# facebookresearch/rela

Hardware: AMD Instinct MI355X
Metric: env-steps/s (Ape-X Atari 84x84x4, actor tick + learner grad-step) (higher is better)
Workload: dtype f32 (f32 operands as 3 exact bf16 parts on bf16 MFMA; f32-accurate); 1 GPU; Ape-X DQN 80x80 envs/GPU, actor+learner on one MI355X, replay 2^20, B=512, A=18, n=3; device-resident static frames; parallelism=single

## Files before the change

### rela_amd/csrc/ffnet.hip

```cpp
#include <atomic>
#include <cstdlib>

#include "common.h"
#include "gemm_bf16s.h"
#include "gemm_f32emu.h"
#include "gemm_s3.h"
#include "conv_img_s3.h"
#include "conv12_s3.h"
#include "ffnet_layout.h"
#include "ffnet_plan.h"
#include "gemm_lds.h"
#include "param_layout.h"
#include "prof.h"

namespace rela_amd {

typedef float f32x4 __attribute__((ext_vector_type(4)));

struct FFNetDev {
  uint4* B1 = nullptr;
  float* b1 = nullptr;
  float *B2 = nullptr, *b2 = nullptr;
  float *B3 = nullptr, *b3 = nullptr;
  float *Bf = nullptr, *bf = nullptr;
// ... 1451 lines not shown
  const int64_t p = (int64_t)blockIdx.x * (blockDim.x >> 6) + (threadIdx.x >> 6);
  if (p >= pixels) return;
  const int c = threadIdx.x & 63;
  uint8_t* r = rec + p * 256;
  const uint16_t hi = reinterpret_cast<const uint16_t*>(r)[c], lo = reinterpret_cast<const uint16_t*>(r)[64 + c];
  const float v = bf16_to_f32(hi) + bf16_to_f32(lo);
  __builtin_amdgcn_wave_barrier();
  asm volatile("s_waitcnt vmcnt(0)" ::: "memory");
  reinterpret_cast<float*>(r)[c] = v;
}

using TileFcSmall = gemm::TileCfg<128, 64, 4, 2, false>;
struct ProbFcFwd : gemm::ProbBase {
  const float *a3, *wt;
  float* part;
  __device__ float4 loadA(int m, int k) const {
    return m < M ? *reinterpret_cast<const float4*>(a3 + (size_t)m * 3136 + k) : make_float4(0.f, 0.f, 0.f, 0.f);
  }
  __device__ float4 loadB(int k, int n) const { return *reinterpret_cast<const float4*>(wt + (size_t)k * 512 + n); }
  __device__ void store(int z, int m, int n, float v) const { part[((size_t)z * M + m) * 512 + n] = v; }
};

__global__ void fc_reduce(const float* __restrict__ part, int splits, int N, const float* __restrict__ bias,
                          float* __restrict__ h) {
  const int idx = blockIdx.x * blockDim.x + threadIdx.x;
  if (idx >= N * 128) return;
  const int n4 = (idx & 127) * 4;
  const size_t off = (size_t)(idx >> 7) * 512 + n4;
  float4 s = *reinterpret_cast<const float4*>(bias + n4);
  for (int z = 0; z < splits; ++z) {
    const float4 v = *reinterpret_cast<const float4*>(part + (size_t)z * N * 512 + off);
    s.x += v.x, s.y += v.y, s.z += v.z, s.w += v.w;
  }
  *reinterpret_cast<float4*>(h + off) =
// ... 1071 lines not shown
```

### rela_amd/csrc/gemm_bf16x3.h

```cpp
#pragma once
#include <hip/hip_runtime.h>

#include <type_traits>

#include "common.h"
#include "gemm_lds.h"
#include "prof.h"

namespace rela_amd {
namespace gemm3 {

typedef float f32x4 __attribute__((ext_vector_type(4)));
typedef float f32x2 __attribute__((ext_vector_type(2)));
typedef __bf16 bf16x8 __attribute__((ext_vector_type(8)));
typedef __bf16 bf16x2 __attribute__((ext_vector_type(2)));
typedef short s16x4 __attribute__((ext_vector_type(4)));
typedef s16x4 __attribute__((address_space(3))) * lds_s16x4_ptr;

constexpr int kT = 512;
constexpr int BK = 32;

__device__ __forceinline__ int krow(int k) {
  const int g = k >> 3, j = k & 7;
  return j < 4 ? 4 * g + j : 16 + 4 * g + (j - 4);
// ... 65 lines not shown
    return bz < gm.gz;
  }
  bx = (i / gm.gy) * 8 + xcd, by = i % gm.gy, bz = 0;
  return bx < gm.gx;
}

template <class T, class P>
__global__ __launch_bounds__(kT) void gemm_bf16x3(const P p, const GridMap gm) {
  extern __shared__ __attribute__((aligned(16))) uint8_t smem[];
  int bx, by, bz;
  if (!grid_map(gm, bx, by, bz)) return;
  const int tid = threadIdx.x;
  const int wave = tid >> 6, lane = tid & 63;
  const int li = lane & 15, g = lane >> 4;
  const int wm = wave / T::WN, wn = wave % T::WN;
  const int m0 = by * T::BM, n0 = bx * T::BN;
  const int nch = (p.K + BK - 1) / BK;
  const int c0 = bz * p.kslice;
  const int c1 = min(nch, c0 + p.kslice);

  constexpr int D = 4;
  float4 ra[D][T::A_IT], rb[D][T::B_IT];
  auto gload = [&](int ch, auto set) {
    constexpr int S = decltype(set)::value;
    const int k0 = ch * BK;
#pragma unroll
    for (int j = 0; j < T::A_IT; ++j) {
      const int idx = min(tid + j * kT, T::A_V4 - 1);
      if constexpr (T::AMC) {
        const int kr = idx / (T::BM / 4), q = idx % (T::BM / 4);
        ra[S][j] = p.loadA(k0 + kr, m0 + 4 * q);
      } else {
        const int r = idx >> 3, q = idx & 7;
        ra[S][j] = p.loadA(m0 + r, k0 + 4 * q);
      }
    }
#pragma unroll
    for (int j = 0; j < T::B_IT; ++j) {
      const int idx = min(tid + j * kT, T::B_V4 - 1);
      const int kr = idx / (T::BN / 4), q = idx % (T::BN / 4);
      rb[S][j] = p.loadB(k0 + kr, n0 + 4 * q);
    }
  };
  auto sstore = [&](int buf, auto set) {
    constexpr int S = decltype(set)::value;
    uint8_t* base = smem + buf * T::BUF;
#pragma unroll
    for (int j = 0; j < T::A_IT; ++j) {
      const int idx = min(tid + j * kT, T::A_V4 - 1);
      uint2 hi, mid, lo;
      if constexpr (T::PARTS == 3) split4x3(ra[S][j], hi, mid, lo);
      else split4(ra[S][j], hi, lo);
      int off;
      if constexpr (T::AMC) {
        const int kr = idx / (T::BM / 4), q = idx % (T::BM / 4);
        off = krow(kr) * T::LDA + q * 8;
      } else {
        const int r = idx >> 3, q = idx & 7;
        off = r * T::LDA + q * 8;
      }
      *reinterpret_cast<uint2*>(base + off) = hi;
      if constexpr (T::PARTS == 3) *reinterpret_cast<uint2*>(base + T::A_HALF + off) = mid;
      *reinterpret_cast<uint2*>(base + (T::PARTS - 1) * T::A_HALF + off) = lo;
    }
    uint8_t* bb = base + T::PARTS * T::A_HALF;
#pragma unroll
    for (int j = 0; j < T::B_IT; ++j) {
      const int idx = min(tid + j * kT, T::B_V4 - 1);
      const int kr = idx / (T::BN / 4), q = idx % (T::BN / 4);
      uint2 hi, mid, lo;
      if constexpr (T::PARTS == 3) split4x3(rb[S][j], hi, mid, lo);
      else split4(rb[S][j], hi, lo);
      const int off = krow(kr) * T::LDB + q * 8;
      *reinterpret_cast<uint2*>(bb + off) = hi;
      if constexpr (T::BPARTS == 3) *reinterpret_cast<uint2*>(bb + T::B_HALF + off) = mid;
      if constexpr (T::BPARTS > 1) *reinterpret_cast<uint2*>(bb + (T::BPARTS - 1) * T::B_HALF + off) = lo;
    }
  };

  const int tr_off = (4 * g + (li >> 2));
  auto frag_tr = [&](const uint8_t* img, int ld, int col0) -> bf16x8 {
    const uint8_t* a0 = img + tr_off * ld + (col0 + 4 * (li & 3)) * 2;
    const s16x4 x = __builtin_amdgcn_ds_read_tr16_b64_v4i16((lds_s16x4_ptr)(a0));
    const s16x4 y = __builtin_amdgcn_ds_read_tr16_b64_v4i16((lds_s16x4_ptr)(a0 + 16 * ld));
    typedef short s16x8 __attribute__((ext_vector_type(8)));
    const s16x8 z = {x[0], x[1], x[2], x[3], y[0], y[1], y[2], y[3]};
    return __builtin_bit_cast(bf16x8, z);
  };
  auto frag_row = [&](const uint8_t* img, int row) -> bf16x8 {
    return __builtin_bit_cast(bf16x8, *reinterpret_cast<const uint4*>(img + row * T::LDA + g * 16));
  };

  f32x4 acc[T::TM][T::TN];
  f32x4 accs[T::PARTS == 3 ? T::TM : 1][T::PARTS == 3 ? T::TN : 1];
#pragma unroll
  for (int t = 0; t < T::TM; ++t)
#pragma unroll
    for (int u = 0; u < T::TN; ++u) {
      acc[t][u] = f32x4{0.f, 0.f, 0.f, 0.f};
      if constexpr (T::PARTS == 3) accs[t][u] = f32x4{0.f, 0.f, 0.f, 0.f};
    }

  using S0 = std::integral_constant<int, 0>;
  using S1 = std::integral_constant<int, 1>;
  using S2 = std::integral_constant<int, 2>;
  using S3 = std::integral_constant<int, 3>;
  if (c0 < c1) gload(c0, S0{});
  if (c0 + 1 < c1) gload(c0 + 1, S1{});
  if (c0 + 2 < c1) gload(c0 + 2, S2{});
  if (c0 + 3 < c1) gload(c0 + 3, S3{});
  if (c0 < c1) sstore(0, S0{});
  __syncthreads();
  auto step = [&](int cur, auto cs, auto ns) {
    const int buf = (cur - c0) & 1;
    if (cur + D < c1) gload(cur + D, cs);
    const uint8_t* base = smem + buf * T::BUF;
    const uint8_t* bb = base + T::PARTS * T::A_HALF;
    bf16x8 bp[T::TN][T::BPARTS];
#pragma unroll
    for (int u = 0; u < T::TN; ++u) {
      const int col0 = (wn * T::TN + u) * 16;
#pragma unroll
      for (int q = 0; q < T::BPARTS; ++q) bp[u][q] = frag_tr(bb + q * T::B_HALF, T::LDB, col0);
    }
#pragma unroll
    for (int t = 0; t < T::TM; ++t) {
      const int row0 = (wm * T::TM + t) * 16;
      bf16x8 ap[T::PARTS];
#pragma unroll
      for (int q = 0; q < T::PARTS; ++q) {
// ... 8 lines not shown
          acc[t][u] = __builtin_amdgcn_mfma_f32_16x16x32_bf16(ap[0], bp[u][0], acc[t][u], 0, 0, 0);
        } else if constexpr (T::BPARTS == 1) {
          accs[t][u] = __builtin_amdgcn_mfma_f32_16x16x32_bf16(ap[2], bp[u][0], accs[t][u], 0, 0, 0);
          accs[t][u] = __builtin_amdgcn_mfma_f32_16x16x32_bf16(ap[1], bp[u][0], accs[t][u], 0, 0, 0);
          acc[t][u] = __builtin_amdgcn_mfma_f32_16x16x32_bf16(ap[0], bp[u][0], acc[t][u], 0, 0, 0);
        } else {
          accs[t][u] = __builtin_amdgcn_mfma_f32_16x16x32_bf16(ap[2], bp[u][0], accs[t][u], 0, 0, 0);
          accs[t][u] = __builtin_amdgcn_mfma_f32_16x16x32_bf16(ap[0], bp[u][2], accs[t][u], 0, 0, 0);
          accs[t][u] = __builtin_amdgcn_mfma_f32_16x16x32_bf16(ap[1], bp[u][1], accs[t][u], 0, 0, 0);
          accs[t][u] = __builtin_amdgcn_mfma_f32_16x16x32_bf16(ap[1], bp[u][0], accs[t][u], 0, 0, 0);
          accs[t][u] = __builtin_amdgcn_mfma_f32_16x16x32_bf16(ap[0], bp[u][1], accs[t][u], 0, 0, 0);
          acc[t][u] = __builtin_amdgcn_mfma_f32_16x16x32_bf16(ap[0], bp[u][0], acc[t][u], 0, 0, 0);
        }
      }
    }
    if (cur + 1 < c1) sstore(buf ^ 1, ns);
    __syncthreads();
  };
  for (int base = c0; base < c1; base += D) {
    step(base, S0{}, S1{});
    if (base + 1 < c1) step(base + 1, S1{}, S2{});
    if (base + 2 < c1) step(base + 2, S2{}, S3{});
    if (base + 3 < c1) step(base + 3, S3{}, S0{});
  }

#pragma unroll
  for (int t = 0; t < T::TM; ++t)
#pragma unroll
    for (int u = 0; u < T::TN; ++u)
#pragma unroll
      for (int r = 0; r < 4; ++r) {
        const int m = m0 + (wm * T::TM + t) * 16 + g * 4 + r;
        const int n = n0 + (wn * T::TN + u) * 16 + li;
        if (m < p.M && n < p.N) {
          if constexpr (T::PARTS == 3) p.store(bz, m, n, acc[t][u][r] + accs[t][u][r]);
          else p.store(bz, m, n, acc[t][u][r]);
        }
      }
}

template <class T, class P>
int launch_gemm(P p, int splits, hipStream_t s, const char* name) {
  static const hipError_t attr_set = hipFuncSetAttribute(reinterpret_cast<const void*>(&gemm_bf16x3<T, P>),
                                                         hipFuncAttributeMaxDynamicSharedMemorySize, T::LDS_BYTES);
  RELA_HIP(attr_set);
  const int nch = ceil_div(p.K, BK);
  p.kslice = ceil_div(nch, splits);
  ProfScope prof(name, s);
// ... 18 lines not shown
```

### rela_amd/csrc/gemm_lds.h

```cpp
#pragma once
#include <hip/hip_runtime.h>

#include <type_traits>

#include "common.h"
#include "prof.h"

namespace rela_amd {
namespace gemm {

typedef float f32x4 __attribute__((ext_vector_type(4)));
constexpr int kLT = 512;
constexpr int BK = 32;

__device__ __forceinline__ float4 zero4() { return make_float4(0.f, 0.f, 0.f, 0.f); }
__device__ __forceinline__ float4 ld4(const float* p) { return *reinterpret_cast<const float4*>(p); }

template <int BM_, int BN_, int WM_, int WN_, bool AMC_>
struct TileCfg {
  static constexpr int BM = BM_, BN = BN_, WM = WM_, WN = WN_;
  static constexpr bool AMC = AMC_;
  static_assert(WM * WN == 8, "8 wavefronts per block");
  static constexpr int TM = BM / 16 / WM, TN = BN / 16 / WN;
  static_assert(TM >= 1 && TN >= 1, "tile too small for the wave grid");
  static constexpr int LDA = AMC ? BM + 16 : BK + 2;
  static constexpr int A_FLOATS = AMC ? BK * LDA : BM * LDA;
  static constexpr int LDB = BN + 16;
  static constexpr int B_FLOATS = BK * LDB;
  static constexpr int A_V4 = BM * BK / 4, B_V4 = BN * BK / 4;
  static constexpr int A_IT = (A_V4 + kLT - 1) / kLT, B_IT = (B_V4 + kLT - 1) / kLT;
};

template <class P, class = void>
struct fold_chunks {
  static constexpr int value = 0;
};
template <class P>
struct fold_chunks<P, std::void_t<decltype(P::kFoldChunks)>> {
  static constexpr int value = P::kFoldChunks;
};

template <class T, class P>
__global__ __launch_bounds__(kLT) void gemm_lds(const P p) {
  __shared__ __attribute__((aligned(16))) float sA[2][T::A_FLOATS];
  __shared__ __attribute__((aligned(16))) float sB[2][T::B_FLOATS];
  const int tid = threadIdx.x;
  const int wave = tid >> 6, lane = tid & 63;
  const int li = lane & 15, kk = lane >> 4;
  const int wm = wave / T::WN, wn = wave % T::WN;
  const int m0 = blockIdx.y * T::BM, n0 = blockIdx.x * T::BN;
  const int nch = (p.K + BK - 1) / BK;
  const int c0 = blockIdx.z * p.kslice;
  const int c1 = min(nch, c0 + p.kslice);

  float4 ra[T::A_IT], rb[T::B_IT];
  auto gload = [&](int ch) {
    const int k0 = ch * BK;
#pragma unroll
    for (int j = 0; j < T::A_IT; ++j) {
      const int idx = tid + j * kLT;
      if (idx < T::A_V4) {
        if constexpr (T::AMC) {
          const int kr = idx / (T::BM / 4), q = idx % (T::BM / 4);
          ra[j] = p.loadA(k0 + kr, m0 + 4 * q);
        } else {
          const int r = idx >> 3, q = idx & 7;
          ra[j] = p.loadA(m0 + r, k0 + 4 * q);
        }
      }
    }
#pragma unroll
    for (int j = 0; j < T::B_IT; ++j) {
      const int idx = tid + j * kLT;
      if (idx < T::B_V4) {
        const int kr = idx / (T::BN / 4), q = idx % (T::BN / 4);
        rb[j] = p.loadB(k0 + kr, n0 + 4 * q);
      }
    }
  };
  auto sstore = [&](int buf) {
#pragma unroll
    for (int j = 0; j < T::A_IT; ++j) {
      const int idx = tid + j * kLT;
      if (idx < T::A_V4) {
        if constexpr (T::AMC) {
          const int kr = idx / (T::BM / 4), q = idx % (T::BM / 4);
          *reinterpret_cast<float4*>(&sA[buf][kr * T::LDA + 4 * q]) = ra[j];
        } else {
          const int r = idx >> 3, q = idx & 7;
          float* d = &sA[buf][r * T::LDA + 4 * q];
          *reinterpret_cast<float2*>(d) = make_float2(ra[j].x, ra[j].y);
          *reinterpret_cast<float2*>(d + 2) = make_float2(ra[j].z, ra[j].w);
        }
      }
    }
#pragma unroll
    for (int j = 0; j < T::B_IT; ++j) {
      const int idx = tid + j * kLT;
      if (idx < T::B_V4) {
        const int kr = idx / (T::BN / 4), q = idx % (T::BN / 4);
        *reinterpret_cast<float4*>(&sB[buf][kr * T::LDB + 4 * q]) = rb[j];
      }
    }
  };

  f32x4 acc[T::TM][T::TN];
#pragma unroll
  for (int t = 0; t < T::TM; ++t)
#pragma unroll
    for (int u = 0; u < T::TN; ++u) acc[t][u] = f32x4{0.f, 0.f, 0.f, 0.f};
  constexpr int FOLD = fold_chunks<P>::value;
  f32x4 tot[FOLD ? T::TM : 1][FOLD ? T::TN : 1];
  if constexpr (FOLD > 0) {
#pragma unroll
    for (int t = 0; t < T::TM; ++t)
#pragma unroll
      for (int u = 0; u < T::TN; ++u) tot[t][u] = f32x4{0.f, 0.f, 0.f, 0.f};
  }

  if (c0 < c1) {
    gload(c0);
    sstore(0);
  }
  __syncthreads();
  for (int ch = c0; ch < c1; ++ch) {
    const int buf = (ch - c0) & 1;
    if (ch + 1 < c1) gload(ch + 1);
#pragma unroll
    for (int ks = 0; ks < BK / 4; ++ks) {
      float a[T::TM], b[T::TN];
#pragma unroll
      for (int t = 0; t < T::TM; ++t) {
        const int row = (wm * T::TM + t) * 16 + li;
        a[t] = T::AMC ? sA[buf][(4 * ks + kk) * T::LDA + row] : sA[buf][row * T::LDA + 4 * ks + kk];
      }
#pragma unroll
      for (int u = 0; u < T::TN; ++u) b[u] = sB[buf][(4 * ks + kk) * T::LDB + (wn * T::TN + u) * 16 + li];
#pragma unroll
      for (int t = 0; t < T::TM; ++t)
#pragma unroll
        for (int u = 0; u < T::TN; ++u) acc[t][u] = __builtin_amdgcn_mfma_f32_16x16x4f32(a[t], b[u], acc[t][u], 0, 0, 0);
    }
    if constexpr (FOLD > 0) {
      if ((ch - c0 + 1) % FOLD == 0) {
#pragma unroll
        for (int t = 0; t < T::TM; ++t)
#pragma unroll
          for (int u = 0; u < T::TN; ++u) {
            tot[t][u] += acc[t][u];
            acc[t][u] = f32x4{0.f, 0.f, 0.f, 0.f};
          }
      }
    }
    if (ch + 1 < c1) sstore(buf ^ 1);
    __syncthreads();
  }

#pragma unroll
  for (int t = 0; t < T::TM; ++t)
#pragma unroll
    for (int u = 0; u < T::TN; ++u)
#pragma unroll
      for (int r = 0; r < 4; ++r) {
        const int m = m0 + (wm * T::TM + t) * 16 + kk * 4 + r;
        const int n = n0 + (wn * T::TN + u) * 16 + li;
        if (m < p.M && n < p.N) {
          if constexpr (FOLD > 0) p.store(blockIdx.z, m, n, tot[t][u][r]);
          else p.store(blockIdx.z, m, n, acc[t][u][r]);
        }
      }
}

struct ProbBase {
  int M, N, K, kslice;
};

template <class T, class P>
void launch_gemm(P p, int splits, hipStream_t s, const char* name) {
  const int nch = ceil_div(p.K, BK);
  p.kslice = ceil_div(nch, splits);
  ProfScope prof(name, s);
  note_launch("gemm_lds (f32)");
  hipLaunchKernelGGL((gemm_lds<T, P>), dim3(ceil_div(p.N, T::BN), ceil_div(p.M, T::BM), splits), dim3(kLT), 0, s, p);
}

}
}
```

### rela_amd/csrc/learner_common.h

```cpp
#pragma once
#include <cmath>
#include <cstring>
#include <vector>

#include "common.h"
#include "ffnet_layout.h"
#include "gemm_lds.h"
#include "gemm_bf16x3.h"
#include "param_layout.h"
#include "prof.h"
#include "value_rescale.h"
#include "dgrad_conv_bf16.h"
#include "wgrad_conv1_bf16.h"
#include "wgrad_conv2_bf16.h"
#include "wgrad_conv3_bf16.h"

namespace rela_amd {
namespace {

using namespace gemm;

using TileDgrad = TileCfg<128, 64, 4, 2, false>;
using TileWfc = TileCfg<128, 64, 4, 2, true>;
using TileW64 = TileCfg<64, 64, 2, 4, true>;
// ... 4 lines not shown
using Tile3Wfc = gemm3::TileCfg<128, 64, 4, 2, true>;
using Tile3W64 = gemm3::TileCfg<64, 64, 2, 4, true>;
using Tile3W32 = gemm3::TileCfg<32, 64, 2, 4, true>;
inline bool gemm_bf16x3_on() { return true; }
using Tile6Dgrad = gemm3::TileCfg<128, 64, 4, 2, false, 3>;
using Tile6Wfc = gemm3::TileCfg<128, 64, 4, 2, true, 3>;
using Tile6W64 = gemm3::TileCfg<64, 64, 2, 4, true, 3>;
using Tile6W32 = gemm3::TileCfg<32, 64, 2, 4, true, 3>;
using Tile6W32U8 = gemm3::SinglePartB<Tile6W32>;


struct ProbHeadDgrad : ProbBase {
  const float *d_ha, *a_w, *v_w, *h;
  float* d_h;
  int A;
  __device__ float4 loadA(int m, int k) const { return m < M ? ld4(d_ha + (size_t)m * 32 + k) : zero4(); }
  __device__ float4 loadB(int k, int n) const {
    if (k < A) return ld4(a_w + (size_t)k * 512 + n);
    if (k == 31) return ld4(v_w + n);
    return zero4();
  }
  __device__ void store(int, int m, int n, float v) const {
    const size_t i = (size_t)m * 512 + n;
    d_h[i] = h[i] > 0.f ? v : 0.f;
  }
};

struct ProbHeadWgradPart : ProbBase {
  const float *d_ha, *h;
  float* part;
  __device__ float4 loadA(int b, int m) const { return b < K ? ld4(d_ha + (size_t)b * 32 + m) : zero4(); }
  __device__ float4 loadB(int b, int n) const { return b < K ? ld4(h + (size_t)b * 512 + n) : zero4(); }
  __device__ void store(int z, int m, int n, float v) const { part[((size_t)z * 32 + m) * 512 + n] = v; }
};
__global__ void head_wgrad_reduce(const float* __restrict__ part, int splits, int A, float* __restrict__ g_a_w,
                                  float* __restrict__ g_v_w) {
  const int idx = blockIdx.x * blockDim.x + threadIdx.x;
  if (idx >= 32 * 512) return;
  const int m = idx >> 9, n = idx & 511;
  if (m >= A && m != 31) return;
  float s = 0.f;
#pragma unroll 8
  for (int z = 0; z < splits; ++z) s += part[(size_t)z * (32 * 512) + idx];
  if (m < A) g_a_w[(size_t)m * 512 + n] = s;
  else g_v_w[n] = s;
}

struct ProbHeadWgrad : ProbBase {
  const float *d_ha, *h;
  float *g_a_w, *g_v_w;
  int A;
  __device__ float4 loadA(int b, int m) const { return b < K ? ld4(d_ha + (size_t)b * 32 + m) : zero4(); }
  __device__ float4 loadB(int b, int n) const { return b < K ? ld4(h + (size_t)b * 512 + n) : zero4(); }
  __device__ void store(int, int m, int n, float v) const {
    if (m < A) g_a_w[(size_t)m * 512 + n] = v;
    else if (m == 31) g_v_w[n] = v;
  }
};

struct ProbFcDgrad : ProbBase {
  const float *d_h, *wfcp, *a3;
  float* d_a3;
  __device__ float4 loadA(int m, int k) const { return m < M ? ld4(d_h + (size_t)m * 512 + k) : zero4(); }
  __device__ float4 loadB(int k, int n) const { return ld4(wfcp + (size_t)k * 3136 + n); }
  __device__ void store(int, int m, int n, float v) const {
    const size_t i = (size_t)m * 3136 + n;
    d_a3[i] = a3[i] > 0.f ? v : 0.f;
  }
};

struct ProbFcWgrad : ProbBase {
  const float *d_h, *a3;
  float* g_fc_w;
  __device__ float4 loadA(int b, int m) const { return b < K ? ld4(d_h + (size_t)b * 512 + m) : zero4(); }
  __device__ float4 loadB(int b, int n) const { return b < K ? ld4(a3 + (size_t)b * 3136 + n) : zero4(); }
  __device__ void store(int, int m, int n, float v) const {
    const int pos = n >> 6, c = n & 63;
    g_fc_w[(size_t)m * 3136 + c * 49 + pos] = v;
  }
};

struct ProbDgrad3 : ProbBase {
  static constexpr int kFoldChunks = 2;
  const float *d_out, *wp, *a2;
  float* d_a2;
  __device__ float4 loadA(int m, int k) const {
    if (m >= M) return zero4();
    const int b = m / 81, pix = m - b * 81;
    const int y = pix / 9, x = pix - y * 9;
    const int tap = k >> 6, oc = k & 63;
    const int kh = tap / 3, kw = tap - kh * 3;
    const int oy = y - kh, ox = x - kw;
    if ((unsigned)oy >= 7u || (unsigned)ox >= 7u) return zero4();
    return ld4(d_out + ((size_t)b * 49 + oy * 7 + ox) * 64 + oc);
  }
  __device__ float4 loadB(int k, int n) const { return ld4(wp + (size_t)(k & 63) * 576 + (k >> 6) * 64 + n); }
  __device__ void store(int, int m, int n, float v) const {
    const size_t i = (size_t)m * 64 + n;
    d_a2[i] = a2[i] > 0.f ? v : 0.f;
  }
};

struct ProbDgrad2 : ProbBase {
  static constexpr int kFoldChunks = 2;
  const float *d_out, *wp, *a1;
  float* d_a1;
  __device__ float4 loadA(int m, int k) const {
    if (m >= M) return zero4();
    const int b = m / 100, pix = m - b * 100;
    const int yh = pix / 10, xh = pix - yh * 10;
    const int t = k >> 6, oc = k & 63;
    const int oy = yh - (t >> 1), ox = xh - (t & 1);
    if ((unsigned)oy >= 9u || (unsigned)ox >= 9u) return zero4();
    return ld4(d_out + ((size_t)b * 81 + oy * 9 + ox) * 64 + oc);
  }
  __device__ float4 loadB(int k, int n) const {
    const int cls = n >> 5, t = k >> 6;
    const int kh = (t & 2) + (cls >> 1), kw = 2 * (t & 1) + (cls & 1);
    return ld4(wp + (size_t)(k & 63) * 512 + (kh * 4 + kw) * 32 + (n & 31));
  }
  __device__ void store(int, int m, int n, float v) const {
    const int cls = n >> 5;
    const int b = m / 100, pix = m - b * 100;
    const int yh = pix / 10, xh = pix - yh * 10;
    const size_t i = ((size_t)b * 400 + (2 * yh + (cls >> 1)) * 20 + 2 * xh + (cls & 1)) * 32 + (n & 31);
    d_a1[i] = a1[i] > 0.f ? v : 0.f;
  }
};

template <int OC, int CIN, int KH, int KW, int STRIDE, int OH, int OW, int IH, int IW>
struct ProbConvWgrad : ProbBase {
  const float *d_out, *in;
  float* part;
  __device__ float4 loadA(int k, int m) const { return k < K ? ld4(d_out + (size_t)k * OC + m) : zero4(); }
  __device__ float4 loadB(int k, int n) const {
    if (k >= K) return zero4();
    const int b = k / (OH * OW), pos = k - b * (OH * OW);
    const int oy = pos / OW, ox = pos - oy * OW;
    const int r = n / CIN, c = n - r * CIN;
    const int kh = r / KW, kw = r - kh * KW;
    return ld4(in + (((size_t)b * IH + oy * STRIDE + kh) * IW + ox * STRIDE + kw) * CIN + c);
  }
  __device__ void store(int z, int m, int n, float v) const { part[((size_t)z * M + m) * N + n] = v; }
};
using ProbW3 = ProbConvWgrad<64, 64, 3, 3, 1, 7, 7, 9, 9>;
using ProbW2 = ProbConvWgrad<64, 32, 4, 4, 2, 9, 9, 20, 20>;

struct ProbW1 : ProbBase {
  const float* d_out;
  const uint8_t* obs;
  float* part;
  __device__ float4 loadA(int k, int m) const { return k < K ? ld4(d_out + (size_t)k * 32 + m) : zero4(); }
  __device__ float4 loadB(int k, int n) const {
    if (k >= K) return zero4();
    const int b = k / 400, pos = k - b * 400;
    const int oy = pos / 20, ox = pos - oy * 20;
    const int c = n >> 6, kh = (n >> 3) & 7, kw = n & 7;
    const uint32_t d = *reinterpret_cast<const uint32_t*>(obs + (size_t)b * 28224 + c * 7056 + (oy * 4 + kh) * 84 +
                                                          ox * 4 + kw);
    return make_float4((float)(d & 0xff), (float)((d >> 8) & 0xff), (float)((d >> 16) & 0xff), (float)(d >> 24));
  }
  __device__ void store(int z, int m, int n, float v) const { part[((size_t)z * M + m) * N + n] = v; }
};


enum { kRedConv1 = 0, kRedConv2 = 1, kRedConv3 = 2 };
__global__ void reduce_splits(const float* __restrict__ part, int splits, int M, int N, int mode,
                              float* __restrict__ out) {
  const int idx = blockIdx.x * blockDim.x + threadIdx.x;
  if (idx >= M * N) return;
  const int m = idx / N, n = idx - m * N;
  float s = 0.f;
#pragma unroll 8
  for (int z = 0; z < splits; ++z) s += part[((size_t)z * M + m) * N + n];
  if (mode == kRedConv1) {
// ... 564 lines not shown
```

### rela_amd/csrc/learner_r2d2.hip

```cpp
#include "gemm_bf16s.h"
#include "learner_common.h"

using namespace rela_amd;

namespace rela_amd {
namespace {

constexpr int kHid = 512, kGates = 2048, kFeat = 3136;
constexpr int kRecSplitF = 4;
constexpr int kRecSplitB = 8;

using TileRows = TileCfg<128, 64, 4, 2, false>;
using TileRec = TileCfg<64, 64, 2, 4, false>;
using TileWg = TileCfg<128, 64, 4, 2, true>;
using TileW32r = TileCfg<32, 64, 2, 4, true>;

struct ProbGateX : ProbBase {
  const float *a3, *wihT, *bias;
  float* gx;
  __device__ float4 loadA(int m, int k) const { return m < M ? ld4(a3 + (size_t)m * kFeat + k) : zero4(); }
  __device__ float4 loadB(int k, int n) const { return ld4(wihT + (size_t)k * kGates + n); }
  __device__ void store(int, int m, int n, float v) const { gx[(size_t)m * kGates + n] = v + bias[n]; }
};
struct ProbRecFwd : ProbBase {
  const float *h, *whhT;
  float* part;
  __device__ float4 loadA(int m, int k) const { return m < M ? ld4(h + (size_t)m * kHid + k) : zero4(); }
  __device__ float4 loadB(int k, int n) const { return ld4(whhT + (size_t)k * kGates + n); }
  __device__ void store(int z, int m, int n, float v) const { part[((size_t)z * M + m) * kGates + n] = v; }
};
struct ProbRecBwd : ProbBase {
  const float *dg, *whh;
  float* part;
  __device__ float4 loadA(int m, int k) const { return m < M ? ld4(dg + (size_t)m * kGates + k) : zero4(); }
  __device__ float4 loadB(int k, int n) const { return ld4(whh + (size_t)k * kHid + n); }
  __device__ void store(int z, int m, int n, float v) const { part[((size_t)z * M + m) * kHid + n] = v; }
};
struct ProbWhh : ProbBase {
  const float *dg, *hprev;
  float* out;
  __device__ float4 loadA(int r, int m) const { return r < K ? ld4(dg + (size_t)r * kGates + m) : zero4(); }
  __device__ float4 loadB(int r, int n) const { return r < K ? ld4(hprev + (size_t)r * kHid + n) : zero4(); }
  __device__ void store(int, int m, int n, float v) const { out[(size_t)m * kHid + n] = v; }
};
struct ProbWih : ProbBase {
  const float *dg, *a3;
  float* out;
  __device__ float4 loadA(int r, int m) const { return r < K ? ld4(dg + (size_t)r * kGates + m) : zero4(); }
  __device__ float4 loadB(int r, int n) const { return r < K ? ld4(a3 + (size_t)r * kFeat + n) : zero4(); }
  __device__ void store(int, int m, int n, float v) const {
    const int pos = n >> 6, c = n & 63;
    out[(size_t)m * kFeat + c * 49 + pos] = v;
  }
};
struct ProbIhDgrad : ProbBase {
  const float *dg, *wihp, *a3;
  float* d_a3;
  __device__ float4 loadA(int m, int k) const { return m < M ? ld4(dg + (size_t)m * kGates + k) : zero4(); }
  __device__ float4 loadB(int k, int n) const { return ld4(wihp + (size_t)k * kFeat + n); }
  __device__ void store(int, int m, int n, float v) const {
    const size_t i = (size_t)m * kFeat + n;
    d_a3[i] = a3[i] > 0.f ? v : 0.f;
  }
};
struct ProbHeadDgradSeq : ProbBase {
  const float *d_ha, *a_w, *v_w;
  float* d_o;
  int A;
  __device__ float4 loadA(int m, int k) const { return m < M ? ld4(d_ha + (size_t)m * 32 + k) : zero4(); }
  __device__ float4 loadB(int k, int n) const {
    if (k < A) return ld4(a_w + (size_t)k * kHid + n);
    if (k == 31) return ld4(v_w + n);
    return zero4();
  }
  __device__ void store(int, int m, int n, float v) const { d_o[(size_t)m * kHid + n] = v; }
};

constexpr int kPackRows = 8;
__global__ __launch_bounds__(256) void pack_lstm_learner(const float* __restrict__ wih, const float* __restrict__ whh,
                                                         const float* __restrict__ bih, const float* __restrict__ bhh,
                                                         float* __restrict__ wihT, float* __restrict__ wihp,
                                                         float* __restrict__ whhT, float* __restrict__ bsum) {
  extern __shared__ __attribute__((aligned(16))) float rows[];
  const int g0 = blockIdx.x * kPackRows, tid = threadIdx.x;
  for (int i = tid; i < kPackRows * kFeat / 4; i += 256)
    reinterpret_cast<float4*>(rows)[i] = reinterpret_cast<const float4*>(wih + (size_t)g0 * kFeat)[i];
  __syncthreads();
  if (wihp) {
    for (int i = tid; i < kPackRows * kFeat; i += 256) {
// ... 1016 lines not shown
```

Measured before the change: 3.488 million env-steps/s.

## Split GEMM operand loads into branch-free fetch and deferred masking with shared chunk ring

Replaces the per-problem loadA/loadB with unconditional clamped fetches plus fix functions that zero out-of-range values at LDS-store time. Global loads can then issue without branches and their latency overlaps the MMA work. Both GEMM kernels now share a templated chunk_ring pipeline with sched barriers; gemm_lds gains a two-deep register ring. The conv1 wgrad problem stages raw uint32 pixels and converts them late. The change costs extra registers and redundant clamped loads at edges.

Result: faster. 3.540 million env-steps/s (median of 6 runs) (+1.5%).

```diff
diff --git a/rela_amd/csrc/ffnet.hip b/rela_amd/csrc/ffnet.hip
--- a/rela_amd/csrc/ffnet.hip
+++ b/rela_amd/csrc/ffnet.hip
@@ -1489,10 +1489,9 @@
 struct ProbFcFwd : gemm::ProbBase {
   const float *a3, *wt;
   float* part;
-  __device__ float4 loadA(int m, int k) const {
-    return m < M ? *reinterpret_cast<const float4*>(a3 + (size_t)m * 3136 + k) : make_float4(0.f, 0.f, 0.f, 0.f);
-  }
-  __device__ float4 loadB(int k, int n) const { return *reinterpret_cast<const float4*>(wt + (size_t)k * 512 + n); }
+  __device__ float4 fetchA(int m, int k) const { return gemm::ld4(a3 + (size_t)min(m, M - 1) * 3136 + k); }
+  __device__ float4 fixA(float4 v, int m, int) const { return gemm::keep4(m < M, v); }
+  __device__ float4 fetchB(int k, int n) const { return gemm::ld4(wt + (size_t)k * 512 + n); }
   __device__ void store(int z, int m, int n, float v) const { part[((size_t)z * M + m) * 512 + n] = v; }
 };
 
diff --git a/rela_amd/csrc/gemm_bf16x3.h b/rela_amd/csrc/gemm_bf16x3.h
--- a/rela_amd/csrc/gemm_bf16x3.h
+++ b/rela_amd/csrc/gemm_bf16x3.h
@@ -103,51 +103,57 @@
   const int wave = tid >> 6, lane = tid & 63;
   const int li = lane & 15, g = lane >> 4;
   const int wm = wave / T::WN, wn = wave % T::WN;
-  const int m0 = by * T::BM, n0 = bx * T::BN;
+  const int bm0 = by * T::BM, bn0 = bx * T::BN;
   const int nch = (p.K + BK - 1) / BK;
   const int c0 = bz * p.kslice;
   const int c1 = min(nch, c0 + p.kslice);
 
   constexpr int D = 4;
-  float4 ra[D][T::A_IT], rb[D][T::B_IT];
+  typename P::StageA ra[D][T::A_IT];
+  typename P::StageB rb[D][T::B_IT];
   auto gload = [&](int ch, auto set) {
     constexpr int S = decltype(set)::value;
-    const int k0 = ch * BK;
+    const int k0 = ch * BK, m0 = bm0, n0 = bn0;
 #pragma unroll
     for (int j = 0; j < T::A_IT; ++j) {
       const int idx = min(tid + j * kT, T::A_V4 - 1);
       if constexpr (T::AMC) {
         const int kr = idx / (T::BM / 4), q = idx % (T::BM / 4);
-        ra[S][j] = p.loadA(k0 + kr, m0 + 4 * q);
+        ra[S][j] = p.fetchA(k0 + kr, m0 + 4 * q);
       } else {
         const int r = idx >> 3, q = idx & 7;
-        ra[S][j] = p.loadA(m0 + r, k0 + 4 * q);
+        ra[S][j] = p.fetchA(m0 + r, k0 + 4 * q);
       }
     }
 #pragma unroll
     for (int j = 0; j < T::B_IT; ++j) {
       const int idx = min(tid + j * kT, T::B_V4 - 1);
       const int kr = idx / (T::BN / 4), q = idx % (T::BN / 4);
-      rb[S][j] = p.loadB(k0 + kr, n0 + 4 * q);
-    }
-  };
-  auto sstore = [&](int buf, auto set) {
+      rb[S][j] = p.fetchB(k0 + kr, n0 + 4 * q);
+    }
+  };
+  auto sstore = [&](int buf, int ch, auto set) {
     constexpr int S = decltype(set)::value;
+    const int z = gemm::store_point();
+    const int k0 = ch * BK + z, m0 = bm0 + z, n0 = bn0 + z;
     uint8_t* base = smem + buf * T::BUF;
 #pragma unroll
     for (int j = 0; j < T::A_IT; ++j) {
       const int idx = min(tid + j * kT, T::A_V4 - 1);
       uint2 hi, mid, lo;
-      if constexpr (T::PARTS == 3) split4x3(ra[S][j], hi, mid, lo);
-      else split4(ra[S][j], hi, lo);
+      float4 v;
       int off;
       if constexpr (T::AMC) {
         const int kr = idx / (T::BM / 4), q = idx % (T::BM / 4);
+        v = p.fixA(ra[S][j], k0 + kr, m0 + 4 * q);
         off = krow(kr) * T::LDA + q * 8;
       } else {
         const int r = idx >> 3, q = idx & 7;
+        v = p.fixA(ra[S][j], m0 + r, k0 + 4 * q);
         off = r * T::LDA + q * 8;
       }
+      if constexpr (T::PARTS == 3) split4x3(v, hi, mid, lo);
+      else split4(v, hi, lo);
       *reinterpret_cast<uint2*>(base + off) = hi;
       if constexpr (T::PARTS == 3) *reinterpret_cast<uint2*>(base + T::A_HALF + off) = mid;
       *reinterpret_cast<uint2*>(base + (T::PARTS - 1) * T::A_HALF + off) = lo;
@@ -158,8 +164,9 @@
       const int idx = min(tid + j * kT, T::B_V4 - 1);
       const int kr = idx / (T::BN / 4), q = idx % (T::BN / 4);
       uint2 hi, mid, lo;
-      if constexpr (T::PARTS == 3) split4x3(rb[S][j], hi, mid, lo);
-      else split4(rb[S][j], hi, lo);
+      const float4 v = p.fixB(rb[S][j], k0 + kr, n0 + 4 * q);
+      if constexpr (T::PARTS == 3) split4x3(v, hi, mid, lo);
+      else split4(v, hi, lo);
       const int off = krow(kr) * T::LDB + q * 8;
       *reinterpret_cast<uint2*>(bb + off) = hi;
       if constexpr (T::BPARTS == 3) *reinterpret_cast<uint2*>(bb + T::B_HALF + off) = mid;
@@ -190,19 +197,7 @@
       if constexpr (T::PARTS == 3) accs[t][u] = f32x4{0.f, 0.f, 0.f, 0.f};
     }
 
-  using S0 = std::integral_constant<int, 0>;
-  using S1 = std::integral_constant<int, 1>;
-  using S2 = std::integral_constant<int, 2>;
-  using S3 = std::integral_constant<int, 3>;
-  if (c0 < c1) gload(c0, S0{});
-  if (c0 + 1 < c1) gload(c0 + 1, S1{});
-  if (c0 + 2 < c1) gload(c0 + 2, S2{});
-  if (c0 + 3 < c1) gload(c0 + 3, S3{});
-  if (c0 < c1) sstore(0, S0{});
-  __syncthreads();
-  auto step = [&](int cur, auto cs, auto ns) {
-    const int buf = (cur - c0) & 1;
-    if (cur + D < c1) gload(cur + D, cs);
+  auto mma = [&](int buf, int) {
     const uint8_t* base = smem + buf * T::BUF;
     const uint8_t* bb = base + T::PARTS * T::A_HALF;
     bf16x8 bp[T::TN][T::BPARTS];
@@ -241,15 +236,8 @@
         }
       }
     }
-    if (cur + 1 < c1) sstore(buf ^ 1, ns);
-    __syncthreads();
-  };
-  for (int base = c0; base < c1; base += D) {
-    step(base, S0{}, S1{});
-    if (base + 1 < c1) step(base + 1, S1{}, S2{});
-    if (base + 2 < c1) step(base + 2, S2{}, S3{});
-    if (base + 3 < c1) step(base + 3, S3{}, S0{});
-  }
+  };
+  if (c0 < c1) gemm::chunk_ring<D>(c0, c1, gload, sstore, mma);
 
 #pragma unroll
   for (int t = 0; t < T::TM; ++t)
@@ -257,8 +245,8 @@
     for (int u = 0; u < T::TN; ++u)
 #pragma unroll
       for (int r = 0; r < 4; ++r) {
-        const int m = m0 + (wm * T::TM + t) * 16 + g * 4 + r;
-        const int n = n0 + (wn * T::TN + u) * 16 + li;
+        const int m = bm0 + (wm * T::TM + t) * 16 + g * 4 + r;
+        const int n = bn0 + (wn * T::TN + u) * 16 + li;
         if (m < p.M && n < p.N) {
           if constexpr (T::PARTS == 3) p.store(bz, m, n, acc[t][u][r] + accs[t][u][r]);
           else p.store(bz, m, n, acc[t][u][r]);
diff --git a/rela_amd/csrc/gemm_lds.h b/rela_amd/csrc/gemm_lds.h
--- a/rela_amd/csrc/gemm_lds.h
+++ b/rela_amd/csrc/gemm_lds.h
@@ -2,6 +2,7 @@
 #include <hip/hip_runtime.h>
 
 #include <type_traits>
+#include <utility>
 
 #include "common.h"
 #include "prof.h"
@@ -15,6 +16,9 @@
 
 __device__ __forceinline__ float4 zero4() { return make_float4(0.f, 0.f, 0.f, 0.f); }
 __device__ __forceinline__ float4 ld4(const float* p) { return *reinterpret_cast<const float4*>(p); }
+__device__ __forceinline__ float4 keep4(bool in_range, float4 v) {
+  return make_float4(in_range ? v.x : 0.f, in_range ? v.y : 0.f, in_range ? v.z : 0.f, in_range ? v.w : 0.f);
+}
 
 template <int BM_, int BN_, int WM_, int WN_, bool AMC_>
 struct TileCfg {
@@ -40,6 +44,50 @@
   static constexpr int value = P::kFoldChunks;
 };
 
+__device__ __forceinline__ int store_point() {
+  int z = 0;
+  asm volatile("" : "+s"(z));
+  return z;
+}
+template <class F, int... I>
+__device__ __forceinline__ void static_for(F&& f, std::integer_sequence<int, I...>) {
+  (f(std::integral_constant<int, I>{}), ...);
+}
+template <int D, class Load, class Store, class Mma>
+__device__ __forceinline__ void chunk_ring(int c0, int c1, Load&& gload, Store&& sstore, Mma&& mma) {
+  using Sets = std::make_integer_sequence<int, D>;
+  static_for([&](auto j) { gload(min(c0 + j.value, c1 - 1), j); }, Sets{});
+  sstore(0, c0, std::integral_constant<int, 0>{});
+  __syncthreads();
+  int base = c0;
+  for (; base + D < c1; base += D) {
+    static_for(
+        [&](auto j) {
+          const int cur = base + j.value, buf = (cur - c0) & 1;
+          gload(min(cur + D, c1 - 1), j);
+          __builtin_amdgcn_sched_barrier(0);
+          mma(buf, cur);
+          __builtin_amdgcn_sched_barrier(0);
+          sstore(buf ^ 1, cur + 1, std::integral_constant<int, (j.value + 1) % D>{});
+          __syncthreads();
+          __builtin_amdgcn_sched_barrier(0);
+        },
+        Sets{});
+  }
+  static_for(
+      [&](auto j) {
+        const int cur = base + j.value, buf = (cur - c0) & 1;
+        if (cur < c1) {
+          mma(buf, cur);
+          if (cur + 1 < c1) sstore(buf ^ 1, cur + 1, std::integral_constant<int, (j.value + 1) % D>{});
+          __syncthreads();
+        }
+      },
+      Sets{});
+}
+
+constexpr int kRing = 2;
+
 template <class T, class P>
 __global__ __launch_bounds__(kLT) void gemm_lds(const P p) {
   __shared__ __attribute__((aligned(16))) float sA[2][T::A_FLOATS];
@@ -48,59 +96,57 @@
   const int wave = tid >> 6, lane = tid & 63;
   const int li = lane & 15, kk = lane >> 4;
   const int wm = wave / T::WN, wn = wave % T::WN;
-  const int m0 = blockIdx.y * T::BM, n0 = blockIdx.x * T::BN;
+  const int bm0 = blockIdx.y * T::BM, bn0 = blockIdx.x * T::BN;
   const int nch = (p.K + BK - 1) / BK;
   const int c0 = blockIdx.z * p.kslice;
   const int c1 = min(nch, c0 + p.kslice);
 
-  float4 ra[T::A_IT], rb[T::B_IT];
-  auto gload = [&](int ch) {
-    const int k0 = ch * BK;
+  typename P::StageA ra[kRing][T::A_IT];
+  typename P::StageB rb[kRing][T::B_IT];
+  auto gload = [&](int ch, auto set) {
+    constexpr int S = decltype(set)::value;
+    const int k0 = ch * BK, m0 = bm0, n0 = bn0;
 #pragma unroll
     for (int j = 0; j < T::A_IT; ++j) {
-      const int idx = tid + j * kLT;
-      if (idx < T::A_V4) {
-        if constexpr (T::AMC) {
-          const int kr = idx / (T::BM / 4), q = idx % (T::BM / 4);
-          ra[j] = p.loadA(k0 + kr, m0 + 4 * q);
-        } else {
-          const int r = idx >> 3, q = idx & 7;
-          ra[j] = p.loadA(m0 + r, k0 + 4 * q);
-        }
+      const int idx = min(tid + j * kLT, T::A_V4 - 1);
+      if constexpr (T::AMC) {
+        const int kr = idx / (T::BM / 4), q = idx % (T::BM / 4);
+        ra[S][j] = p.fetchA(k0 + kr, m0 + 4 * q);
+      } else {
+        const int r = idx >> 3, q = idx & 7;
+        ra[S][j] = p.fetchA(m0 + r, k0 + 4 * q);
       }
     }
 #pragma unroll
     for (int j = 0; j < T::B_IT; ++j) {
-      const int idx = tid + j * kLT;
-      if (idx < T::B_V4) {
-        const int kr = idx / (T::BN / 4), q = idx % (T::BN / 4);
-        rb[j] = p.loadB(k0 + kr, n0 + 4 * q);
-      }
+      const int idx = min(tid + j * kLT, T::B_V4 - 1);
+      const int kr = idx / (T::BN / 4), q = idx % (T::BN / 4);
+      rb[S][j] = p.fetchB(k0 + kr, n0 + 4 * q);
     }
   };
-  auto sstore = [&](int buf) {
+  auto sstore = [&](int buf, int ch, auto set) {
+    constexpr int S = decltype(set)::value;
+    const int z = store_point();
+    const int k0 = ch * BK + z, m0 = bm0 + z, n0 = bn0 + z;
 #pragma unroll
     for (int j = 0; j < T::A_IT; ++j) {
-      const int idx = tid + j * kLT;
-      if (idx < T::A_V4) {
-        if constexpr (T::AMC) {
-          const int kr = idx / (T::BM / 4), q = idx % (T::BM / 4);
-          *reinterpret_cast<float4*>(&sA[buf][kr * T::LDA + 4 * q]) = ra[j];
-        } else {
-          const int r = idx >> 3, q = idx & 7;
-          float* d = &sA[buf][r * T::LDA + 4 * q];
-          *reinterpret_cast<float2*>(d) = make_float2(ra[j].x, ra[j].y);
-          *reinterpret_cast<float2*>(d + 2) = make_float2(ra[j].z, ra[j].w);
-        }
+      const int idx = min(tid + j * kLT, T::A_V4 - 1);
+      if constexpr (T::AMC) {
+        const int kr = idx / (T::BM / 4), q = idx % (T::BM / 4);
+        *reinterpret_cast<float4*>(&sA[buf][kr * T::LDA + 4 * q]) = p.fixA(ra[S][j], k0 + kr, m0 + 4 * q);
+      } else {
+        const int r = idx >> 3, q = idx & 7;
+        const float4 v = p.fixA(ra[S][j], m0 + r, k0 + 4 * q);
+        float* d = &sA[buf][r * T::LDA + 4 * q];
+        *reinterpret_cast<float2*>(d) = make_float2(v.x, v.y);
+        *reinterpret_cast<float2*>(d + 2) = make_float2(v.z, v.w);
       }
     }
 #pragma unroll
     for (int j = 0; j < T::B_IT; ++j) {
-      const int idx = tid + j * kLT;
-      if (idx < T::B_V4) {
-        const int kr = idx / (T::BN / 4), q = idx % (T::BN / 4);
-        *reinterpret_cast<float4*>(&sB[buf][kr * T::LDB + 4 * q]) = rb[j];
-      }
+      const int idx = min(tid + j * kLT, T::B_V4 - 1);
+      const int kr = idx / (T::BN / 4), q = idx % (T::BN / 4);
+      *reinterpret_cast<float4*>(&sB[buf][kr * T::LDB + 4 * q]) = p.fixB(rb[S][j], k0 + kr, n0 + 4 * q);
     }
   };
 
@@ -118,14 +164,7 @@
       for (int u = 0; u < T::TN; ++u) tot[t][u] = f32x4{0.f, 0.f, 0.f, 0.f};
   }
 
-  if (c0 < c1) {
-    gload(c0);
-    sstore(0);
-  }
-  __syncthreads();
-  for (int ch = c0; ch < c1; ++ch) {
-    const int buf = (ch - c0) & 1;
-    if (ch + 1 < c1) gload(ch + 1);
+  auto mma = [&](int buf, int ch) {
 #pragma unroll
     for (int ks = 0; ks < BK / 4; ++ks) {
       float a[T::TM], b[T::TN];
@@ -152,9 +191,8 @@
           }
       }
     }
-    if (ch + 1 < c1) sstore(buf ^ 1);
-    __syncthreads();
-  }
+  };
+  if (c0 < c1) chunk_ring<kRing>(c0, c1, gload, sstore, mma);
 
 #pragma unroll
   for (int t = 0; t < T::TM; ++t)
@@ -162,8 +200,8 @@
     for (int u = 0; u < T::TN; ++u)
 #pragma unroll
       for (int r = 0; r < 4; ++r) {
-        const int m = m0 + (wm * T::TM + t) * 16 + kk * 4 + r;
-        const int n = n0 + (wn * T::TN + u) * 16 + li;
+        const int m = bm0 + (wm * T::TM + t) * 16 + kk * 4 + r;
+        const int n = bn0 + (wn * T::TN + u) * 16 + li;
         if (m < p.M && n < p.N) {
           if constexpr (FOLD > 0) p.store(blockIdx.z, m, n, tot[t][u][r]);
           else p.store(blockIdx.z, m, n, acc[t][u][r]);
@@ -173,6 +211,10 @@
 
 struct ProbBase {
   int M, N, K, kslice;
+  using StageA = float4;
+  using StageB = float4;
+  __device__ float4 fixA(float4 v, int, int) const { return v; }
+  __device__ float4 fixB(float4 v, int, int) const { return v; }
 };
 
 template <class T, class P>
diff --git a/rela_amd/csrc/learner_common.h b/rela_amd/csrc/learner_common.h
--- a/rela_amd/csrc/learner_common.h
+++ b/rela_amd/csrc/learner_common.h
@@ -42,12 +42,13 @@
   const float *d_ha, *a_w, *v_w, *h;
   float* d_h;
   int A;
-  __device__ float4 loadA(int m, int k) const { return m < M ? ld4(d_ha + (size_t)m * 32 + k) : zero4(); }
-  __device__ float4 loadB(int k, int n) const {
-    if (k < A) return ld4(a_w + (size_t)k * 512 + n);
-    if (k == 31) return ld4(v_w + n);
-    return zero4();
-  }
+  __device__ float4 fetchA(int m, int k) const { return ld4(d_ha + (size_t)min(m, M - 1) * 32 + k); }
+  __device__ float4 fixA(float4 v, int m, int) const { return keep4(m < M, v); }
+  __device__ float4 fetchB(int k, int n) const {
+    const float* row = k < A ? a_w + (size_t)k * 512 : v_w;
+    return ld4(row + n);
+  }
+  __device__ float4 fixB(float4 v, int k, int) const { return keep4(k < A || k == 31, v); }
   __device__ void store(int, int m, int n, float v) const {
     const size_t i = (size_t)m * 512 + n;
     d_h[i] = h[i] > 0.f ? v : 0.f;
@@ -57,8 +58,10 @@
 struct ProbHeadWgradPart : ProbBase {
   const float *d_ha, *h;
   float* part;
-  __device__ float4 loadA(int b, int m) const { return b < K ? ld4(d_ha + (size_t)b * 32 + m) : zero4(); }
-  __device__ float4 loadB(int b, int n) const { return b < K ? ld4(h + (size_t)b * 512 + n) : zero4(); }
+  __device__ float4 fetchA(int b, int m) const { return ld4(d_ha + (size_t)min(b, K - 1) * 32 + m); }
+  __device__ float4 fetchB(int b, int n) const { return ld4(h + (size_t)min(b, K - 1) * 512 + n); }
+  __device__ float4 fixA(float4 v, int b, int) const { return keep4(b < K, v); }
+  __device__ float4 fixB(float4 v, int b, int) const { return keep4(b < K, v); }
   __device__ void store(int z, int m, int n, float v) const { part[((size_t)z * 32 + m) * 512 + n] = v; }
 };
 __global__ void head_wgrad_reduce(const float* __restrict__ part, int splits, int A, float* __restrict__ g_a_w,
@@ -78,8 +81,10 @@
   const float *d_ha, *h;
   float *g_a_w, *g_v_w;
   int A;
-  __device__ float4 loadA(int b, int m) const { return b < K ? ld4(d_ha + (size_t)b * 32 + m) : zero4(); }
-  __device__ float4 loadB(int b, int n) const { return b < K ? ld4(h + (size_t)b * 512 + n) : zero4(); }
+  __device__ float4 fetchA(int b, int m) const { return ld4(d_ha + (size_t)min(b, K - 1) * 32 + m); }
+  __device__ float4 fetchB(int b, int n) const { return ld4(h + (size_t)min(b, K - 1) * 512 + n); }
+  __device__ float4 fixA(float4 v, int b, int) const { return keep4(b < K, v); }
+  __device__ float4 fixB(float4 v, int b, int) const { return keep4(b < K, v); }
   __device__ void store(int, int m, int n, float v) const {
     if (m < A) g_a_w[(size_t)m * 512 + n] = v;
     else if (m == 31) g_v_w[n] = v;
@@ -89,8 +94,9 @@
 struct ProbFcDgrad : ProbBase {
   const float *d_h, *wfcp, *a3;
   float* d_a3;
-  __device__ float4 loadA(int m, int k) const { return m < M ? ld4(d_h + (size_t)m * 512 + k) : zero4(); }
-  __device__ float4 loadB(int k, int n) const { return ld4(wfcp + (size_t)k * 3136 + n); }
+  __device__ float4 fetchA(int m, int k) const { return ld4(d_h + (size_t)min(m, M - 1) * 512 + k); }
+  __device__ float4 fixA(float4 v, int m, int) const { return keep4(m < M, v); }
+  __device__ float4 fetchB(int k, int n) const { return ld4(wfcp + (size_t)k * 3136 + n); }
   __device__ void store(int, int m, int n, float v) const {
     const size_t i = (size_t)m * 3136 + n;
     d_a3[i] = a3[i] > 0.f ? v : 0.f;
@@ -100,8 +106,10 @@
 struct ProbFcWgrad : ProbBase {
   const float *d_h, *a3;
   float* g_fc_w;
-  __device__ float4 loadA(int b, int m) const { return b < K ? ld4(d_h + (size_t)b * 512 + m) : zero4(); }
-  __device__ float4 loadB(int b, int n) const { return b < K ? ld4(a3 + (size_t)b * 3136 + n) : zero4(); }
+  __device__ float4 fetchA(int b, int m) const { return ld4(d_h + (size_t)min(b, K - 1) * 512 + m); }
+  __device__ float4 fetchB(int b, int n) const { return ld4(a3 + (size_t)min(b, K - 1) * 3136 + n); }
+  __device__ float4 fixA(float4 v, int b, int) const { return keep4(b < K, v); }
+  __device__ float4 fixB(float4 v, int b, int) const { return keep4(b < K, v); }
   __device__ void store(int, int m, int n, float v) const {
     const int pos = n >> 6, c = n & 63;
     g_fc_w[(size_t)m * 3136 + c * 49 + pos] = v;
@@ -112,17 +120,25 @@
   static constexpr int kFoldChunks = 2;
   const float *d_out, *wp, *a2;
   float* d_a2;
-  __device__ float4 loadA(int m, int k) const {
-    if (m >= M) return zero4();
-    const int b = m / 81, pix = m - b * 81;
-    const int y = pix / 9, x = pix - y * 9;
-    const int tap = k >> 6, oc = k & 63;
-    const int kh = tap / 3, kw = tap - kh * 3;
-    const int oy = y - kh, ox = x - kw;
-    if ((unsigned)oy >= 7u || (unsigned)ox >= 7u) return zero4();
-    return ld4(d_out + ((size_t)b * 49 + oy * 7 + ox) * 64 + oc);
-  }
-  __device__ float4 loadB(int k, int n) const { return ld4(wp + (size_t)(k & 63) * 576 + (k >> 6) * 64 + n); }
+  __device__ void tap_pixel(int m, int k, int& b, int& oy, int& ox) const {
+    m = min(m, M - 1);
+    b = m / 81;
+    const int pix = m - b * 81, y = pix / 9, x = pix - y * 9;
+    const int tap = k >> 6, kh = tap / 3, kw = tap - kh * 3;
+    oy = y - kh, ox = x - kw;
+  }
+  __device__ float4 fetchA(int m, int k) const {
+    int b, oy, ox;
+    tap_pixel(m, k, b, oy, ox);
+    oy = min(max(oy, 0), 6), ox = min(max(ox, 0), 6);
+    return ld4(d_out + ((size_t)b * 49 + oy * 7 + ox) * 64 + (k & 63));
+  }
+  __device__ float4 fixA(float4 v, int m, int k) const {
+    int b, oy, ox;
+    tap_pixel(m, k, b, oy, ox);
+    return keep4(m < M && (unsigned)oy < 7u && (unsigned)ox < 7u, v);
+  }
+  __device__ float4 fetchB(int k, int n) const { return ld4(wp + (size_t)(k & 63) * 576 + (k >> 6) * 64 + n); }
   __device__ void store(int, int m, int n, float v) const {
     const size_t i = (size_t)m * 64 + n;
     d_a2[i] = a2[i] > 0.f ? v : 0.f;
@@ -133,16 +149,25 @@
   static constexpr int kFoldChunks = 2;
   const float *d_out, *wp, *a1;
   float* d_a1;
-  __device__ float4 loadA(int m, int k) const {
-    if (m >= M) return zero4();
-    const int b = m / 100, pix = m - b * 100;
-    const int yh = pix / 10, xh = pix - yh * 10;
-    const int t = k >> 6, oc = k & 63;
-    const int oy = yh - (t >> 1), ox = xh - (t & 1);
-    if ((unsigned)oy >= 9u || (unsigned)ox >= 9u) return zero4();
-    return ld4(d_out + ((size_t)b * 81 + oy * 9 + ox) * 64 + oc);
-  }
-  __device__ float4 loadB(int k, int n) const {
+  __device__ void tap_pixel(int m, int k, int& b, int& oy, int& ox) const {
+    m = min(m, M - 1);
+    b = m / 100;
+    const int pix = m - b * 100, yh = pix / 10, xh = pix - yh * 10;
+    const int t = k >> 6;
+    oy = yh - (t >> 1), ox = xh - (t & 1);
+  }
+  __device__ float4 fetchA(int m, int k) const {
+    int b, oy, ox;
+    tap_pixel(m, k, b, oy, ox);
+    oy = min(max(oy, 0), 8), ox = min(max(ox, 0), 8);
+    return ld4(d_out + ((size_t)b * 81 + oy * 9 + ox) * 64 + (k & 63));
+  }
+  __device__ float4 fixA(float4 v, int m, int k) const {
+    int b, oy, ox;
+    tap_pixel(m, k, b, oy, ox);
+    return keep4(m < M && (unsigned)oy < 9u && (unsigned)ox < 9u, v);
+  }
+  __device__ float4 fetchB(int k, int n) const {
     const int cls = n >> 5, t = k >> 6;
     const int kh = (t & 2) + (cls >> 1), kw = 2 * (t & 1) + (cls & 1);
     return ld4(wp + (size_t)(k & 63) * 512 + (kh * 4 + kw) * 32 + (n & 31));
@@ -160,9 +185,11 @@
 struct ProbConvWgrad : ProbBase {
   const float *d_out, *in;
   float* part;
-  __device__ float4 loadA(int k, int m) const { return k < K ? ld4(d_out + (size_t)k * OC + m) : zero4(); }
-  __device__ float4 loadB(int k, int n) const {
-    if (k >= K) return zero4();
+  __device__ float4 fetchA(int k, int m) const { return ld4(d_out + (size_t)min(k, K - 1) * OC + m); }
+  __device__ float4 fixA(float4 v, int k, int) const { return keep4(k < K, v); }
+  __device__ float4 fixB(float4 v, int k, int) const { return keep4(k < K, v); }
+  __device__ float4 fetchB(int k, int n) const {
+    k = min(k, K - 1);
     const int b = k / (OH * OW), pos = k - b * (OH * OW);
     const int oy = pos / OW, ox = pos - oy * OW;
     const int r = n / CIN, c = n - r * CIN;
@@ -178,15 +205,19 @@
   const float* d_out;
   const uint8_t* obs;
   float* part;
-  __device__ float4 loadA(int k, int m) const { return k < K ? ld4(d_out + (size_t)k * 32 + m) : zero4(); }
-  __device__ float4 loadB(int k, int n) const {
-    if (k >= K) return zero4();
+  using StageB = uint32_t;
+  __device__ float4 fetchA(int k, int m) const { return ld4(d_out + (size_t)min(k, K - 1) * 32 + m); }
+  __device__ float4 fixA(float4 v, int k, int) const { return keep4(k < K, v); }
+  __device__ uint32_t fetchB(int k, int n) const {
+    k = min(k, K - 1);
     const int b = k / 400, pos = k - b * 400;
     const int oy = pos / 20, ox = pos - oy * 20;
     const int c = n >> 6, kh = (n >> 3) & 7, kw = n & 7;
-    const uint32_t d = *reinterpret_cast<const uint32_t*>(obs + (size_t)b * 28224 + c * 7056 + (oy * 4 + kh) * 84 +
-                                                          ox * 4 + kw);
-    return make_float4((float)(d & 0xff), (float)((d >> 8) & 0xff), (float)((d >> 16) & 0xff), (float)(d >> 24));
+    return *reinterpret_cast<const uint32_t*>(obs + (size_t)b * 28224 + c * 7056 + (oy * 4 + kh) * 84 + ox * 4 + kw);
+  }
+  __device__ float4 fixB(uint32_t d, int k, int) const {
+    return keep4(k < K,
+                 make_float4((float)(d & 0xff), (float)((d >> 8) & 0xff), (float)((d >> 16) & 0xff), (float)(d >> 24)));
   }
   __device__ void store(int z, int m, int n, float v) const { part[((size_t)z * M + m) * N + n] = v; }
 };
diff --git a/rela_amd/csrc/learner_r2d2.hip b/rela_amd/csrc/learner_r2d2.hip
--- a/rela_amd/csrc/learner_r2d2.hip
+++ b/rela_amd/csrc/learner_r2d2.hip
@@ -18,36 +18,43 @@
 struct ProbGateX : ProbBase {
   const float *a3, *wihT, *bias;
   float* gx;
-  __device__ float4 loadA(int m, int k) const { return m < M ? ld4(a3 + (size_t)m * kFeat + k) : zero4(); }
-  __device__ float4 loadB(int k, int n) const { return ld4(wihT + (size_t)k * kGates + n); }
+  __device__ float4 fetchA(int m, int k) const { return ld4(a3 + (size_t)min(m, M - 1) * kFeat + k); }
+  __device__ float4 fixA(float4 v, int m, int) const { return keep4(m < M, v); }
+  __device__ float4 fetchB(int k, int n) const { return ld4(wihT + (size_t)k * kGates + n); }
   __device__ void store(int, int m, int n, float v) const { gx[(size_t)m * kGates + n] = v + bias[n]; }
 };
 struct ProbRecFwd : ProbBase {
   const float *h, *whhT;
   float* part;
-  __device__ float4 loadA(int m, int k) const { return m < M ? ld4(h + (size_t)m * kHid + k) : zero4(); }
-  __device__ float4 loadB(int k, int n) const { return ld4(whhT + (size_t)k * kGates + n); }
+  __device__ float4 fetchA(int m, int k) const { return ld4(h + (size_t)min(m, M - 1) * kHid + k); }
+  __device__ float4 fixA(float4 v, int m, int) const { return keep4(m < M, v); }
+  __device__ float4 fetchB(int k, int n) const { return ld4(whhT + (size_t)k * kGates + n); }
   __device__ void store(int z, int m, int n, float v) const { part[((size_t)z * M + m) * kGates + n] = v; }
 };
 struct ProbRecBwd : ProbBase {
   const float *dg, *whh;
   float* part;
-  __device__ float4 loadA(int m, int k) const { return m < M ? ld4(dg + (size_t)m * kGates + k) : zero4(); }
-  __device__ float4 loadB(int k, int n) const { return ld4(whh + (size_t)k * kHid + n); }
+  __device__ float4 fetchA(int m, int k) const { return ld4(dg + (size_t)min(m, M - 1) * kGates + k); }
+  __device__ float4 fixA(float4 v, int m, int) const { return keep4(m < M, v); }
+  __device__ float4 fetchB(int k, int n) const { return ld4(whh + (size_t)k * kHid + n); }
   __device__ void store(int z, int m, int n, float v) const { part[((size_t)z * M + m) * kHid + n] = v; }
 };
 struct ProbWhh : ProbBase {
   const float *dg, *hprev;
   float* out;
-  __device__ float4 loadA(int r, int m) const { return r < K ? ld4(dg + (size_t)r * kGates + m) : zero4(); }
-  __device__ float4 loadB(int r, int n) const { return r < K ? ld4(hprev + (size_t)r * kHid + n) : zero4(); }
+  __device__ float4 fetchA(int r, int m) const { return ld4(dg + (size_t)min(r, K - 1) * kGates + m); }
+  __device__ float4 fixA(float4 v, int r, int) const { return keep4(r < K, v); }
+  __device__ float4 fetchB(int r, int n) const { return ld4(hprev + (size_t)min(r, K - 1) * kHid + n); }
+  __device__ float4 fixB(float4 v, int r, int) const { return keep4(r < K, v); }
   __device__ void store(int, int m, int n, float v) const { out[(size_t)m * kHid + n] = v; }
 };
 struct ProbWih : ProbBase {
   const float *dg, *a3;
   float* out;
-  __device__ float4 loadA(int r, int m) const { return r < K ? ld4(dg + (size_t)r * kGates + m) : zero4(); }
-  __device__ float4 loadB(int r, int n) const { return r < K ? ld4(a3 + (size_t)r * kFeat + n) : zero4(); }
+  __device__ float4 fetchA(int r, int m) const { return ld4(dg + (size_t)min(r, K - 1) * kGates + m); }
+  __device__ float4 fixA(float4 v, int r, int) const { return keep4(r < K, v); }
+  __device__ float4 fetchB(int r, int n) const { return ld4(a3 + (size_t)min(r, K - 1) * kFeat + n); }
+  __device__ float4 fixB(float4 v, int r, int) const { return keep4(r < K, v); }
   __device__ void store(int, int m, int n, float v) const {
     const int pos = n >> 6, c = n & 63;
     out[(size_t)m * kFeat + c * 49 + pos] = v;
@@ -56,8 +63,9 @@
 struct ProbIhDgrad : ProbBase {
   const float *dg, *wihp, *a3;
   float* d_a3;
-  __device__ float4 loadA(int m, int k) const { return m < M ? ld4(dg + (size_t)m * kGates + k) : zero4(); }
-  __device__ float4 loadB(int k, int n) const { return ld4(wihp + (size_t)k * kFeat + n); }
+  __device__ float4 fetchA(int m, int k) const { return ld4(dg + (size_t)min(m, M - 1) * kGates + k); }
+  __device__ float4 fixA(float4 v, int m, int) const { return keep4(m < M, v); }
+  __device__ float4 fetchB(int k, int n) const { return ld4(wihp + (size_t)k * kFeat + n); }
   __device__ void store(int, int m, int n, float v) const {
     const size_t i = (size_t)m * kFeat + n;
     d_a3[i] = a3[i] > 0.f ? v : 0.f;
@@ -67,12 +75,13 @@
   const float *d_ha, *a_w, *v_w;
   float* d_o;
   int A;
-  __device__ float4 loadA(int m, int k) const { return m < M ? ld4(d_ha + (size_t)m * 32 + k) : zero4(); }
-  __device__ float4 loadB(int k, int n) const {
-    if (k < A) return ld4(a_w + (size_t)k * kHid + n);
-    if (k == 31) return ld4(v_w + n);
-    return zero4();
-  }
+  __device__ float4 fetchA(int m, int k) const { return ld4(d_ha + (size_t)min(m, M - 1) * 32 + k); }
+  __device__ float4 fixA(float4 v, int m, int) const { return keep4(m < M, v); }
+  __device__ float4 fetchB(int k, int n) const {
+    const float* row = k < A ? a_w + (size_t)k * kHid : v_w;
+    return ld4(row + n);
+  }
+  __device__ float4 fixB(float4 v, int k, int) const { return keep4(k < A || k == 31, v); }
   __device__ void store(int, int m, int n, float v) const { d_o[(size_t)m * kHid + n] = v; }
 };
 
```
